# jcjones/ct-mapreduce

Hardware: AMD Instinct MI355X
Metric: certificates/sec whole-node + achieved HBM GB/s, 100M-entry synthetic CT batch (higher is better)
Workload: dtype u8

## Files before the change

ct_mapreduce_amd/csrc/der_walk.h:

```cpp
#pragma once
#include <stdint.h>

#include <type_traits>
#include <utility>

#if defined(__HIPCC__)
#define CTMR_HD __host__ __device__ __forceinline__
#else
#define CTMR_HD inline
#endif

namespace ctmr {

struct Walk {
  uint32_t serial_off, serial_len;
  int64_t not_before, not_after;
  uint32_t cn_off, cn_len;
  uint32_t spki_off, spki_len;
  bool bc_valid, is_ca;
  uint32_t nonfatal;
  uint32_t serial_w[5];
  bool cn_match;
  uint32_t meta_issuer, meta_crl;
  uint32_t issuer_name, subject_name;
// ... 1371 lines not shown
    uint32_t d0 = 0, d1 = 0;
    o.subject_name = q;
    q = walk_name<false, STRINGS>(r, L, q, tbs_end, ok, d0, d1, o.nonfatal, strings);
#endif
  }
  if constexpr (NAMES_ONLY) return ok;
  CTMR_STAGE(4);
  touch_all(r, q, SPKI_HEAD_NEED);
  rd_hdr(r, L, q, tbs_end, ok, tag, cs, ce);
  ok = ok & (tag == 0x30u);
  o.spki_off = q;
  o.spki_len = ce - q;
  AlgView key_alg{0u, 0u, 0u, 0u, 0u, 0u};
  KeyPending key_pending;
  key_pending.alg = PK_OTHER;
  {
    uint32_t k, tk, ck, ek;
    alg_id(r, L, cs, ce, ok, k, key_alg);
    rd_hdr(r, L, k, ce, ok, tk, ck, ek);
    ok = ok & (tk == 0x03u);
    bit_string_check(r, L, ck, ek - ck, ok);
    if (spki) spki_key_begin(r, L, key_alg, ck, ek, ok, o.nonfatal, key_pending);
  }
  q = ce;
  r.touch_tail(q, tbs_end);
  if (spki) {
    key_tail_of(r, q, key_pending);
    EcPending ecp;
    spki_key_finish<EC_DEFER>(r, L, key_alg, key_pending, ok, o.nonfatal, ecp);
    o.ec_curve = ecp.curve; o.ec_pos = ecp.pos; o.ec_shift = ecp.shift;
  }
  CTMR_STAGE(5);
  uint32_t nt = 0u;
  uint32_t san_cv = 0u, san_ev = 0u;
  (void)san_cv; (void)san_ev;
  if (ok & (q < tbs_end)) {
    rd_hdr<false>(r, L, q, tbs_end, ok, tag, cs, ce);
    nt = ok ? tag : 0u;
  }
  if (nt == 0x81u) {
    ok = ok & (ce <= tbs_end);
    bit_string_check(r, L, cs, ce - cs, ok);
    q = ce;
    nt = 0u;
    if (ok & (q < tbs_end)) {
      rd_hdr<false>(r, L, q, tbs_end, ok, tag, cs, ce);
      nt = ok ? tag : 0u;
    }
  }
  if (nt == 0x82u) {
    ok = ok & (ce <= tbs_end);
    bit_string_check(r, L, cs, ce - cs, ok);
    q = ce;
    nt = 0u;
    if (ok & (q < tbs_end)) {
      rd_hdr<false>(r, L, q, tbs_end, ok, tag, cs, ce);
      nt = ok ? tag : 0u;
    }
  }
  if ((nt == 0xa3u) | (nt == 0x83u)) ok = ok & (ce != cs);
  if (ok & (nt == 0xa3u)) {
    uint32_t e, e_end;
    r.touch(q, 48);
    rd_hdr<false>(r, L, cs, tbs_end, ok, tag, e, e_end);
    ok = ok & ((tag != 0x30u) | (e_end <= tbs_end));
    e_end = tag == 0x30u ? e_end : e;
    while (ok & (e < e_end)) {
      uint32_t t1, x, x_end, to, co, eo, tv, cv, ev, oidw;
      r.touch(e, 16);
      const uint32_t w0 = ldc(r, e, L), w1 = ldc(r, e + 4u, L), w2 = ldc(r, e + 8u, L);
      const bool p0 = ((w0 & 0xffff80ffu) == 0x03060030u) & ((w1 & 0x808080u) == 0u);
      const uint32_t b7 = w1 >> 24, b9 = (w2 >> 8) & 0xffu;
      const bool nc = p0 & (b7 == 0x04u) & ((w2 & 0x80u) == 0u);
      const bool cr = p0 & (b7 == 0x01u) & ((w2 & 0x80ff00ffu) == 0x00040001u) & ((b9 == 0x00u) | (b9 == 0xffu));
      if (nc | cr) {
        x_end = e + 2u + ((w0 >> 8) & 0xffu);
        co = e + 4u;
        eo = e + 7u;
        oidw = w1;
        cv = e + (cr ? 12u : 9u);
        ev = cv + (cr ? (w2 >> 24) : (w2 & 0xffu));
        ok = ok & (x_end <= e_end) & (ev <= x_end);
      } else {
        r.touch(e, 24);
        rd_hdr(r, L, e, e_end, ok, t1, x, x_end);
        rd_hdr(r, L, x, x_end, ok, to, co, eo);
        oidw = ldc(r, co, L);
        rd_hdr(r, L, eo, x_end, ok, tv, cv, ev);
        ok = ok & (t1 == 0x30u) & (to == 0x06u);
        ok = ok && oid_arcs_ok(r, L, co, eo);
        if (tv == 0x01u) {
          const uint32_t bv = ldc(r, cv, L) & 0xffu;
          ok = ok & (ev - cv == 1u) & ((bv == 0x00u) | (bv == 0xffu));
          rd_hdr(r, L, ev, x_end, ok, tv, cv, ev);
        }
        ok = ok & (tv == 0x04u);
      }
      {
        const bool is_crl = (eo - co == 3u) & ((oidw & 0xffffffu) == 0x1f1d55u);
        const uint32_t pk = o.meta_crl == META_NONE ? meta_pack(cv, ev - cv) : META_HOST;
        o.meta_crl = is_crl ? pk : o.meta_crl;
      }
      if constexpr (STRINGS) {
        if (ext & ok) {
          const uint32_t kind = ext_kind(eo - co, oidw, ldc(r, co + 4u, L));
          if ((kind >= 1u) & (kind <= 6u)) {
            ext_body_check(r, L, kind, cv, ev, ok);
          } else if (kind == 7u) {
            if constexpr (has_coop_refill<R>::value) {
              if ((san_ev == 0u) & (ev > cv)) { san_cv = cv; san_ev = ev; }
              else ext_san_check(r, L, cv, ev, ok, o.nonfatal);
            } else {
              ext_san_check(r, L, cv, ev, ok, o.nonfatal);
            }
          } else if (kind == 9u) {
            uint32_t uo[1] = {0u}, ul[1] = {0u}, nu = 0u;
            r.touch(cv, ev - cv < 200u ? ev - cv : 200u);
            crl_dps<false, true, STRINGS, 1u>(r, L, cv, ev, ok, uo, ul, nu, o.nonfatal, strings);
          } else if (kind == 8u) {
            if constexpr (has_defer_exact<R>::value) r.defer_exact();
            else ext_nc_check(r, L, cv, ev, ok);
          } else if ((kind >= 12u) & ext_nf) {
            if constexpr (has_defer_exact<R>::value) r.defer_exact();
            else o.nonfatal = (kind == 12u ? ext_ipaddr_ok(r, L, cv, ev) : ext_asnum_ok(r, L, cv, ev)) ? o.nonfatal : (o.nonfatal | WALK_NF_EXT);
          } else if ((kind == 10u) & ext_nf && ((ldc(r, co + 8u, L) & 0xffffu) == 0x0204u)) {
            if constexpr (has_defer_exact<R>::value) r.defer_exact();
            else o.nonfatal = ext_sct_ok(r, L, cv, ev) ? o.nonfatal : (o.nonfatal | WALK_NF_EXT);
          }
        }
      }
      if (ok & (eo - co == 3u) & ((oidw & 0xffffffu) == 0x131d55u)) {
        uint32_t tb, c, c_end, tf = 0u, cf = 0u, ef = 0u;
        rd_hdr(r, L, cv, ev, ok, tb, c, c_end);
        ok = ok & (tb == 0x30u) & (c_end == ev);
        bool ca = false;
        if (ok & (c < c_end)) {
          rd_hdr<false>(r, L, c, c_end, ok, tf, cf, ef);
          if (tf == 0x01u) {
            const uint32_t bv = ldc(r, cf, L) & 0xffu;
            ok = ok & (ef <= c_end) & (ef - cf == 1u) & ((bv == 0x00u) | (bv == 0xffu));
            ca = bv == 0xffu;
            c = ef;
            tf = 0u;
            if (ok & (c < c_end)) rd_hdr<false>(r, L, c, c_end, ok, tf, cf, ef);
          }
          if (ok & (c < c_end) & (tf == 0x02u)) {
            ok = ok & (ef <= c_end);
            int32_check(r, L, cf, ef - cf, ok, o.nonfatal);
          }
        }
        o.bc_valid = true;
        o.is_ca = ca;
      }
      e = x_end;
    }
  }
  if constexpr (STRINGS && has_coop_refill<R>::value) {
    if (ext) ext_san_coop(r, L, san_cv, ok ? san_ev : 0u, ok, o.nonfatal);
  }
  CTMR_STAGE(6);
  if constexpr (!TBS_ONLY) {
    const TailView<R> tv{r};
    uint32_t sq;
    alg_id(tv, L, tbs_end, L, ok, sq);
    rd_hdr(tv, L, sq, L, ok, tag, cs, ce);
    ok = ok & (tag == 0x03u);
    bit_string_check(tv, L, cs, ce - cs, ok);
// ... 19 lines not shown
```

ct_mapreduce_amd/csrc/engine/map.inc:

```

int ctmr_set_filter(ctmr_engine* e, const char* filter, size_t len, int log_expired, int64_t now) {
  if (!e || (len && !filter)) return CTMR_E_INVAL;
  std::lock_guard<std::mutex> g(e->mu);
  HIPCHK(e, hipSetDevice(e->device));
  FilterDev f;
  memset(&f, 0, sizeof f);
  f.active = len != 0;
  f.log_expired = log_expired != 0;
  f.now = now;
  f.strict_spki = e->strict_spki ? 1u : 0u;
  f.strict_strings = e->strict_strings ? 1u : 0u;
  f.strict_ext = e->strict_ext ? 1u : 0u;
  size_t s = 0;
  uint32_t nw = 0;
  for (;;) {
    size_t t = s;
    while (t < len && filter[t] != ',') t++;
    const size_t pl = t - s;
    if (f.n_pieces >= 64 || nw + (pl + 3) / 4 > 1024)
      return fail(e, CTMR_E_INVAL, "issuerCNFilter too large (max 64 pieces / 4096 bytes)");
    f.piece_len[f.n_pieces] = (uint32_t)pl;
    f.piece_word[f.n_pieces] = nw;
    memcpy((uint8_t*)(f.words + nw), filter + s, pl);
    nw += (uint32_t)((pl + 3) / 4);
// ... 36 lines not shown
  if (variant == 15 && !fuse) variant = 13;
  const dim3 grid((unsigned)((n + 63) / 64));
#ifdef CTMR_SWEEP
  static const size_t extra_lds = getenv("CTMR_EXTRA_LDS") ? (size_t)atoi(getenv("CTMR_EXTRA_LDS")) : 0;
#else
  constexpr size_t extra_lds = 0;
#endif
  const bool strict = e->strict_strings || e->strict_ext;
  if (variant == 15) {
    MetaCheck mc{};
    XchgArgs xa{};
    if (xchg) xa = *xchg;
    bool meta = false;
    if (e->cfg.collect_meta && e->d_meta_slots) {
      mc.slots = e->d_meta_slots; mc.mask = e->n_meta_slots - 1; mc.arena = e->d_meta_arena;
      mc.hour_pages = e->d_meta_hour_pages; mc.n_hour_pages = e->d_meta_hour_pages ? (uint32_t)e->meta_hour_pages.size() : 0u;
      mc.refs = e->d_meta_refs; mc.n_refs = e->max_issuers;
      mc.enabled = 1;
      meta = true;
      e->meta_precheck_n = first + n;
      e->meta_precheck_ent = fuse->ent - first;
    }
#define CTMR_LAUNCH_FUSED(META, MODE)                                                                                        \
  do {                                                                                                                       \
    if (strict)                                                                                                              \
      hipLaunchKernelGGL((k_map_fused<WIN_CH_STRICT, META, MODE, true>), grid, dim3(64),                                     \
                         WinGeo<WIN_CH_STRICT>::LDS_BYTES + extra_lds, e->stream, ma, *fuse, mc, xa);                        \
    else                                                                                                                     \
      hipLaunchKernelGGL((k_map_fused<WIN_CH_FAST, META, MODE, false>), grid, dim3(64),                                      \
                         WinGeo<WIN_CH_FAST>::LDS_BYTES + extra_lds, e->stream, ma, *fuse, mc, xa);                          \
  } while (0)
    if (mode == XM_OWNER) { if (meta) CTMR_LAUNCH_FUSED(true, XM_OWNER); else CTMR_LAUNCH_FUSED(false, XM_OWNER); }
    else if (mode == XM_BLOOM) { if (meta) CTMR_LAUNCH_FUSED(true, XM_BLOOM); else CTMR_LAUNCH_FUSED(false, XM_BLOOM); }
    else { if (meta) CTMR_LAUNCH_FUSED(true, XM_LOCAL); else CTMR_LAUNCH_FUSED(false, XM_LOCAL); }
#undef CTMR_LAUNCH_FUSED
  } else if (variant == 13) {
    if (strict) hipLaunchKernelGGL((k_map_winc<WIN_CH_STRICT, true>), grid, dim3(64), WinGeo<WIN_CH_STRICT>::LDS_BYTES + extra_lds, e->stream, ma);
    else hipLaunchKernelGGL((k_map_winc<WIN_CH_FAST, false>), grid, dim3(64), WinGeo<WIN_CH_FAST>::LDS_BYTES + extra_lds, e->stream, ma);
#ifdef CTMR_SWEEP
  } else if (variant == 2) {
    hipLaunchKernelGGL(k_map_direct, dim3((unsigned)((n + 255) / 256)), dim3(256), 0, e->stream, ma);
  } else if (variant == 1 && !d_ends) {
    uint32_t C = e->cfg.certs_per_tile ? e->cfg.certs_per_tile : 32;
    if (C > 64) C = 64;
    uint32_t lds = e->cfg.lds_tile_bytes ? e->cfg.lds_tile_bytes : 65536;
    if (lds > 160 * 1024) lds = 160 * 1024;
    ma.certs_per_tile = C; ma.lds_bytes = lds;
    if (!e->tile_attr_set) {
      HIPCHK(e, hipFuncSetAttribute((const void*)k_map_tile, hipFuncAttributeMaxDynamicSharedMemorySize, 160 * 1024));
      e->tile_attr_set = true;
    }
    hipLaunchKernelGGL(k_map_tile, dim3((unsigned)((n + C - 1) / C)), dim3(64), lds, e->stream, ma);
#endif
  } else {
    return fail(e, CTMR_E_INVAL, "map_variant %u is not built into this library", variant);
  }
  return CTMR_OK;
}

static bool round_fused(const ctmr_engine* e) { return e->cfg.map_variant == 0 || e->cfg.map_variant == 15; }

static void round_insert_args(ctmr_engine* e, const RoundCtx& rc, InsertArgs& ia) {
  ia.records = rc.d_records; ia.payload = rc.d_payload; ia.offsets = rc.d_offsets; ia.ends = rc.d_ends; ia.canon = e->d_canon;
  ia.t = e->tbl(); ia.ref0 = rc.ref0; ia.slot_id = (uint32_t*)e->d_scratch[SC_SLOTID];
  ia.ent = (uint32_t*)e->d_scratch[SC_ENT]; ia.n = rc.n; ia.stats = e->d_stats; ia.ord_base = rc.ord_base;
  ia.keypos = (const unsigned long long*)e->d_scratch[SC_KEYPOS]; ia.stage = nullptr; ia.bloom = nullptr; ia.bloom_wmask = 0;
}

static int round_prepare(ctmr_engine* e, RoundCtx& rc) {
  HIPCHK(e, hipSetDevice(e->device));
  e->rd.valid = false;
  const uint64_t n = rc.n;
  if (n >= 0xfffffff0ull) return fail(e, CTMR_E_INVAL, "batch too large (n < 2^32-16)");
  if (((uintptr_t)rc.d_payload & 15) != 0) return fail(e, CTMR_E_INVAL, "payload must be 16-byte aligned");
  int r;
  if (!rc.d_records) {
    if ((r = ensure(e, SC_RECORDS, n * sizeof(ctmr_record)))) return r;
    rc.d_records = (ctmr_record*)e->d_scratch[SC_RECORDS];
  }
  const uint64_t nb = (n + 1023) / 1024;
  if ((r = ensure(e, SC_SLOTID, n * 4))) return r;
  if ((r = ensure(e, SC_ENT, n * 4))) return r;
  if ((r = ensure(e, SC_BLKNEW, nb * 4))) return r;
  if ((r = ensure(e, SC_BLKBASE, nb * 8))) return r;
  if (e->strict_spki && n && (r = ensure(e, SC_KEYPOS, n * 8))) return r;
  if (e->cfg.collect_meta && (r = ensure(e, SC_META, n * 8))) return r;
  if ((r = ensure_capacity(e, n, true))) return r;
  rc.ref0 = e->arena_used;
  e->arena_used += n;
  e->epoch++;
  e->pairs_dirty = true;
  HIPCHK(e, hipMemsetAsync(e->d_stats, 0, 2 * sizeof(DevStats), e->stream));
  const bool fused = round_fused(e);
  if (!fused && rc.mode == XM_OWNER) return fail(e, CTMR_E_INVAL, "the owner-computes exchange needs the fused map kernel (map_variant 0 / 15)");
  if (rc.mode == XM_LOCAL && fused && e->d_bloom) {
    rc.mode = XM_BLOOM;
  }
  if (rc.mode == XM_BLOOM && !e->d_bloom) return fail(e, CTMR_E_INVAL, "ctmr_bloom_config has not been called");
  return CTMR_OK;
}

static int round_launch_range(ctmr_engine* e, RoundCtx& rc, const XchgArgs* xchg, uint64_t lo, uint64_t hi) {
  const uint64_t n = hi - lo;
  if (!n) return CTMR_OK;
  const bool prof = e->cfg.profile != 0;
  int r;
  InsertArgs ia;
  round_insert_args(e, rc, ia);
  ia.records += lo; ia.offsets += lo; ia.slot_id += lo; ia.ent += lo; ia.n = n; ia.ref0 += lo; ia.ord_base += (uint32_t)lo;
  if (ia.ends) ia.ends += lo;
  if (ia.keypos) ia.keypos += lo;
  const bool fused = round_fused(e);
  XchgArgs xa{};
  if (xchg) xa = *xchg;
  if (xa.stage) xa.stage += lo;
  if (xa.wave_cnt) xa.wave_cnt += (lo / 64) * MAX_WORLD;
  if (rc.mode == XM_BLOOM) {
    xa.bloom = e->d_bloom;
    xa.bloom_wmask = e->bloom_words - 1;
  }
  if (prof && lo == 0) HIPCHK(e, hipEventRecord(e->ev[0], e->stream));
  const int kmode = !fused ? XM_LOCAL : (rc.mode == XM_OWNER && rc.world == 1) ? XM_LOCAL : rc.mode;
  if ((r = launch_map(e, rc.d_payload, rc.d_offsets + lo, rc.d_issuer_idx + lo, rc.d_entry_type ? rc.d_entry_type + lo : nullptr, n,
                      rc.d_records + lo, true, fused ? &ia : nullptr, rc.d_ends ? rc.d_ends + lo : nullptr,
                      rc.blob_bytes + CTMR_PAYLOAD_PAD, kmode, &xa, lo)))
    return r;
  if (prof && hi == rc.n) HIPCHK(e, hipEventRecord(e->ev[1], e->stream));
  if (!fused) hipLaunchKernelGGL(k_insert, dim3((unsigned)((n + 255) / 256)), dim3(256), 0, e->stream, ia);
  if (e->strict_spki) {
    ia.stage = (kmode == XM_OWNER) ? xa.stage : nullptr;
    ia.bloom = (rc.mode == XM_BLOOM && fused) ? xa.bloom : nullptr;
    ia.bloom_wmask = xa.bloom_wmask;
    hipLaunchKernelGGL(k_ec_resolve<true>, dim3((unsigned)((n + EC_PER_BLOCK - 1) / EC_PER_BLOCK)), dim3(256), 0, e->stream, ia, rc.d_records + lo);
    hipLaunchKernelGGL(k_ec_resolve<false>, dim3((unsigned)((n + EC_PER_BLOCK - 1) / EC_PER_BLOCK)), dim3(256), 0, e->stream, ia, rc.d_records + lo);
  }
  hipLaunchKernelGGL(k_insert2, dim3((unsigned)((n + INSERT2_PER_BLOCK - 1) / INSERT2_PER_BLOCK)), dim3(256), 0, e->stream, ia, rc.d_records + lo);
  if (!fused && rc.mode == XM_BLOOM)
    hipLaunchKernelGGL(k_bloom_add, dim3((unsigned)((n + 255) / 256)), dim3(256), 0, e->stream, ia, e->d_bloom, e->bloom_words - 1);
  if (prof && hi == rc.n) HIPCHK(e, hipEventRecord(e->ev[2], e->stream));
  return CTMR_OK;
}

static int round_begin(ctmr_engine* e, RoundCtx& rc, const XchgArgs* xchg) {
  int r;
  if ((r = round_prepare(e, rc))) return r;
  return round_launch_range(e, rc, xchg, 0, rc.n);
}

static void round_compact(ctmr_engine* e, const RoundCtx& rc) {
  const uint64_t nb = (rc.n + 1023) / 1024;
  uint32_t* d_blk_new = (uint32_t*)e->d_scratch[SC_BLKNEW];
  uint64_t* d_blk_base = (uint64_t*)e->d_scratch[SC_BLKBASE];
  hipLaunchKernelGGL(k_scan_blocks, dim3(1), dim3(1024), 0, e->stream, d_blk_new, nb, d_blk_base);
  hipLaunchKernelGGL(k_compact, dim3((unsigned)nb), dim3(256), 0, e->stream, (const ctmr_record*)rc.d_records,
                     (const uint32_t*)e->d_scratch[SC_ENT], rc.n, (const uint64_t*)d_blk_base, rc.d_new_idx);
}

static int round_resolve(ctmr_engine* e, RoundCtx& rc, bool compact_now) {
  const bool prof = e->cfg.profile != 0;
  const uint64_t nb = (rc.n + 1023) / 1024;
  ResolveArgs ra;
  ra.ent = (uint32_t*)e->d_scratch[SC_ENT]; ra.issuer_counts = e->issuer_counts; ra.stats = e->d_stats;
  ra.blk_new = (uint32_t*)e->d_scratch[SC_BLKNEW]; ra.n = rc.n;
  hipLaunchKernelGGL(k_resolve, dim3((unsigned)(nb < 512 ? nb : 512)), dim3(1024), 0, e->stream, ra, nb);
  if (prof) HIPCHK(e, hipEventRecord(e->ev[3], e->stream));
  rc.compacted = false;
  if (compact_now && rc.d_new_idx) {
    round_compact(e, rc);
    rc.compacted = true;
  }
  if (prof) HIPCHK(e, hipEventRecord(e->ev[4], e->stream));
  return CTMR_OK;
}

static int round_collect(ctmr_engine* e, RoundCtx& rc) {
  const uint64_t n = rc.n;
  uint32_t* d_ent = (uint32_t*)e->d_scratch[SC_ENT];
  uint32_t* d_blk_new = (uint32_t*)e->d_scratch[SC_BLKNEW];
  DevStats both[2];
  uint64_t ends[2] = {0, rc.blob_bytes};
  HIPCHK(e, hipMemcpyAsync(both, e->d_stats, sizeof both, hipMemcpyDeviceToHost, e->stream));
  if (!rc.d_ends && rc.payload_bytes_known == ~0ull) {
    HIPCHK(e, hipMemcpyAsync(&ends[0], rc.d_offsets, 8, hipMemcpyDeviceToHost, e->stream));
    HIPCHK(e, hipMemcpyAsync(&ends[1], rc.d_offsets + n, 8, hipMemcpyDeviceToHost, e->stream));
  } else if (!rc.d_ends) {
    ends[1] = rc.payload_bytes_known;
  }
  HIPCHK(e, hipStreamSynchronize(e->stream));
  HIPCHK(e, hipGetLastError());
  rc.hs = both[0];
  rc.remote_new = both[1].n_new;
  rc.payload_bytes = ends[1] - ends[0];
  e->occupied += (rc.own_counted ? 0ull : rc.hs.n_new - rc.hs.n_remote) + rc.remote_new;
  if (rc.hs.n_full || both[1].n_full)
    return fail(e, CTMR_E_FULL, "known-certificate table full (%llu slots): %llu entries dropped",
                (unsigned long long)e->nslots, rc.hs.n_full + both[1].n_full);

  rc.host_new = 0;
  rc.host_list.clear();
  if (rc.hs.n_host) {
    std::vector<uint32_t> ent(n);
    HIPCHK(e, hipMemcpy(ent.data(), d_ent, n * 4, hipMemcpyDeviceToHost));
    for (uint64_t i = 0; i < n; i++) {
      if (((ent[i] >> 3) & 7u) != ES_HOST) continue;
      uint64_t off[2];
      ctmr_record rec;
      HIPCHK(e, hipMemcpy(off, rc.d_offsets + i, rc.d_ends ? 8 : 16, hipMemcpyDeviceToHost));
      if (rc.d_ends) HIPCHK(e, hipMemcpy(off + 1, rc.d_ends + i, 8, hipMemcpyDeviceToHost));
      HIPCHK(e, hipMemcpy(&rec, rc.d_records + i, sizeof rec, hipMemcpyDeviceToHost));
      std::vector<uint8_t> der(off[1] - off[0] + 32);
      HIPCHK(e, hipMemcpy(der.data(), rc.d_payload + off[0], off[1] - off[0], hipMemcpyDeviceToHost));
      HostReader hr{der.data()};
      Walk w;
      if (!walk_cert(hr, (uint32_t)(off[1] - off[0]), w, nullptr, e->strict_spki)) continue;
      const uint32_t canon = e->issuers[rec.issuer_idx].canon;
      std::string key = make_key(e, rec.exp_hour, canon);
      std::string member((const char*)der.data() + w.serial_off, w.serial_len);
      if (e->hstore[key].insert(member).second) {
        rc.host_new++;
        e->host_issuer_counts[canon]++;
        rc.host_list.push_back({i, rec.exp_hour, canon, member});
        uint8_t fl = rec.flags | CTMR_FL_WAS_UNKNOWN;
        HIPCHK(e, hipMemcpy((uint8_t*)(rc.d_records + i) + 1, &fl, 1, hipMemcpyHostToDevice));
        const uint32_t en = (ent[i] & ~(7u << 3)) | (ES_CLAIMED << 3);
        HIPCHK(e, hipMemcpy(d_ent + i, &en, 4, hipMemcpyHostToDevice));
        uint32_t bn;
        HIPCHK(e, hipMemcpy(&bn, d_blk_new + i / 1024, 4, hipMemcpyDeviceToHost));
        bn++;
        HIPCHK(e, hipMemcpy(d_blk_new + i / 1024, &bn, 4, hipMemcpyHostToDevice));
      }
    }
    if (rc.host_new && rc.compacted) {
      round_compact(e, rc);
      HIPCHK(e, hipStreamSynchronize(e->stream));
      HIPCHK(e, hipGetLastError());
    }
  }
  return CTMR_OK;
}

static int round_host_drop(ctmr_engine* e, RoundCtx& rc, const std::vector<size_t>& which) {
  if (which.empty()) return CTMR_OK;
  uint32_t* d_ent = (uint32_t*)e->d_scratch[SC_ENT];
  uint32_t* d_blk_new = (uint32_t*)e->d_scratch[SC_BLKNEW];
  for (size_t idx : which) {
    const RoundCtx::HostNew& h = rc.host_list[idx];
    const std::string key = make_key(e, h.exp_hour, h.canon);
    auto it = e->hstore.find(key);
    if (it != e->hstore.end()) {
      it->second.erase(h.member);
      if (it->second.empty()) e->hstore.erase(it);
    }
    auto ic = e->host_issuer_counts.find(h.canon);
// ... 112 lines not shown
```

ct_mapreduce_amd/csrc/kernels/readers.h:

```cpp
#pragma once
#include "../ctmr_dev.h"
#include "../entry_decode.h"
#include "../synth.h"

namespace ctmr {

struct __attribute__((packed, aligned(1))) U16t { uint32_t a, b, c, d; };

typedef uint32_t ctmr_u32x4 __attribute__((ext_vector_type(4)));
__device__ __forceinline__ uint4 ld_payload16(const uint4* p) {
  const ctmr_u32x4 t = __builtin_nontemporal_load((const ctmr_u32x4*)p);
  return make_uint4(t.x, t.y, t.z, t.w);
}
__device__ __forceinline__ void st_stream16(uint4* p, const uint4& v) {
  ctmr_u32x4 t;
  t.x = v.x; t.y = v.y; t.z = v.z; t.w = v.w;
  __builtin_nontemporal_store(t, (ctmr_u32x4*)p);
}
extern __shared__ __attribute__((aligned(16))) uint8_t smem[];
#ifndef CTMR_WIN_CH_FAST
#define CTMR_WIN_CH_FAST 13
#endif
#ifndef CTMR_WIN_CH_STRICT
#define CTMR_WIN_CH_STRICT 14
#endif
constexpr int WIN_CH_FAST = CTMR_WIN_CH_FAST, WIN_CH_STRICT = CTMR_WIN_CH_STRICT;
#ifndef CTMR_SAN_ALIGN
#define CTMR_SAN_ALIGN 32u
#endif
#ifndef CTMR_WIN_XDW14
#define CTMR_WIN_XDW14 0u
#endif
template <int WCH>
struct WinGeo {
  static constexpr uint32_t XDW = WCH == 13 ? 2u : WCH == 14 ? CTMR_WIN_XDW14 : 0u;
  static constexpr uint32_t WBYTES = (uint32_t)WCH * 16u + XDW * 4u;
  static constexpr uint32_t STRIDE = WCH == 16 ? 272u : WCH == 15 ? 248u : WCH == 13 ? 220u : (uint32_t)WCH * 16u + 12u;
#ifdef CTMR_WIN_NO_SKIP
  static constexpr uint32_t SKIP = 0u;
#else
  static constexpr uint32_t SKIP = WCH == 13 ? 8u : 0u;
#endif
  static constexpr uint32_t LDS_BYTES = 64u * STRIDE;
  static constexpr uint32_t ALIGN = STRIDE % 16u == 0u ? 16u : STRIDE % 8u == 0u ? 8u : 4u;
};
constexpr uint32_t WIN_LDS_MAX = WinGeo<WIN_CH_STRICT>::LDS_BYTES > WinGeo<WIN_CH_FAST>::LDS_BYTES ? WinGeo<WIN_CH_STRICT>::LDS_BYTES
                                                                                               : WinGeo<WIN_CH_FAST>::LDS_BYTES;
template <int WCH>
__device__ __forceinline__ uint32_t win_off(uint32_t c) { return c * WinGeo<WCH>::STRIDE; }
typedef uint32_t ctmr_u32x4_a16 __attribute__((ext_vector_type(4), aligned(16)));
typedef uint32_t ctmr_u32x4_a8 __attribute__((ext_vector_type(4), aligned(8)));
typedef uint32_t ctmr_u32x4_a4 __attribute__((ext_vector_type(4), aligned(4)));
typedef uint32_t ctmr_u32x2_a4 __attribute__((ext_vector_type(2), aligned(4)));
template <int WCH>
__device__ __forceinline__ void st_chunk(uint8_t* at, const uint4& v) {
  using vec_t = typename std::conditional<WinGeo<WCH>::ALIGN == 16u, ctmr_u32x4_a16,
                                          typename std::conditional<WinGeo<WCH>::ALIGN == 8u, ctmr_u32x4_a8, ctmr_u32x4_a4>::type>::type;
  vec_t t;
  t.x = v.x; t.y = v.y; t.z = v.z; t.w = v.w;
  *(vec_t*)at = t;
}
template <int WCH>
__device__ __forceinline__ void st_part(uint8_t* at, const uint4& v) {
  if constexpr (WinGeo<WCH>::XDW == 2u) {
    ctmr_u32x2_a4 t;
    t.x = v.x; t.y = v.y;
    *(ctmr_u32x2_a4*)at = t;
  } else if constexpr (WinGeo<WCH>::XDW == 1u) {
    *(uint32_t*)at = v.x;
  } else if constexpr (WinGeo<WCH>::XDW == 3u) {
    ctmr_u32x2_a4 t;
    t.x = v.x; t.y = v.y;
    *(ctmr_u32x2_a4*)at = t;
    *(uint32_t*)(at + 8) = v.z;
  }
}
__device__ __forceinline__ void st_half(uint8_t* at, uint32_t x, uint32_t y) {
  ctmr_u32x2_a4 t;
  t.x = x; t.y = y;
  *(ctmr_u32x2_a4*)at = t;
}
template <int WCH>
constexpr uint32_t win_loaders() { return (uint32_t)WCH + (WinGeo<WCH>::XDW ? 1u : 0u); }

constexpr uint32_t REL_NONE = 0x80000000u;
constexpr uint64_t REL_SPAN = 0x7e000000ull;
struct WaveBuf {
  __amdgpu_buffer_rsrc_t rs;
  uint64_t b128;
};
__device__ __forceinline__ WaveBuf wave_buf(const uint8_t* payload, uint64_t limit, uint64_t lo0) {
  const uint32_t l = __builtin_amdgcn_readfirstlane((uint32_t)lo0), h = __builtin_amdgcn_readfirstlane((uint32_t)(lo0 >> 32));
  const uint64_t b128 = (((uint64_t)h << 32) | l) & ~127ull;
  uint64_t span = limit > b128 ? limit - b128 : 0ull;
  span = span > 0x7fffffffull ? 0x7fffffffull : span;
  return WaveBuf{__builtin_amdgcn_make_buffer_rsrc((void*)(payload + b128), 0, (int)span, 0x00020000), b128};
}
__device__ __forceinline__ uint32_t wave_rel(const WaveBuf& wb, uint64_t lo, bool has) {
  const uint64_t d = lo - wb.b128;
  return (has & (lo >= wb.b128) & (d < REL_SPAN)) ? (uint32_t)d : REL_NONE;
}
template <bool NT = true>
__device__ __forceinline__ uint4 ld_chunk(const WaveBuf& wb, uint32_t off) {
  const ctmr_u32x4 t = __builtin_amdgcn_raw_buffer_load_b128(wb.rs, (int)off, 0, NT ? 2  : 0);
  return make_uint4(t.x, t.y, t.z, t.w);
}

// ... 311 lines not shown
```

ct_mapreduce_amd/csrc/kernels/reduce.h:

```cpp
#pragma once
#include "keyrec.h"
#include "map.h"

namespace ctmr {

#define AGENT __HIP_MEMORY_SCOPE_AGENT

__device__ __forceinline__ unsigned long long ld_agent(const unsigned long long* p) {
  return __hip_atomic_load(p, __ATOMIC_RELAXED, AGENT);
}
__device__ __forceinline__ void st_agent(unsigned long long* p, unsigned long long v) {
  __hip_atomic_store(p, v, __ATOMIC_RELAXED, AGENT);
}

__device__ __forceinline__ bool cell_equals(const KeyCell* c, unsigned long long meta, const unsigned long long s[5]) {
  bool eq = (ld_agent(&c->meta) & ~CELL_SHADOW) == meta;
#pragma unroll
  for (int k = 0; k < 5; k++) eq = eq && ld_agent(&c->s[k]) == s[k];
  return eq;
}
__device__ __forceinline__ void cell_write(KeyCell* c, unsigned long long meta, const unsigned long long s[5], uint32_t ord) {
  uint4* q = (uint4*)c;
  q[0] = make_uint4((uint32_t)meta, (uint32_t)(meta >> 32), (uint32_t)s[0], (uint32_t)(s[0] >> 32));
  q[1] = make_uint4((uint32_t)s[1], (uint32_t)(s[1] >> 32), (uint32_t)s[2], (uint32_t)(s[2] >> 32));
// ... 487 lines not shown
      const uint4 r0 = rp[0], r1 = rp[1];
      bool good;
      if constexpr (P256) {
        good = ec_point_bits<CurveP256>((const uint32_t*)a.payload, xbit);
      } else {
        switch (curve) {
          case 2u: good = ec_point_bits<CurveP384>((const uint32_t*)a.payload, xbit); break;
          case 3u: good = ec_point_bits<CurveP521>((const uint32_t*)a.payload, xbit); break;
          case 4u: good = ec_point_bits<CurveP224>((const uint32_t*)a.payload, xbit); break;
          default: good = ec_point_bits<CurveP192>((const uint32_t*)a.payload, xbit); break;
        }
      }
      if (!good) {
        const uint32_t stn = (r0.x & 0xffu) == CTMR_ST_ENTRY_DECODE_ERROR ? (uint32_t)CTMR_ST_ENTRY_DECODE_ERROR : (uint32_t)CTMR_ST_PARSE_ERROR;
        rp[0] = make_uint4(stn | (((r0.x >> 8) & CTMR_FL_PRECERT) << 8), 0u, r0.z, 0u);
        rp[1] = make_uint4(0u, 0u, 0u, 0u);
        if ((kp >> 38) & 1ull) {
          a.stage[(i & ~63ull) + ((kp >> 39) & 63ull)].meta = 0ull;
        } else if (ent_state(e) == ES_REMOTE) {
          atomicAdd(&a.stats->n_xl, ~0ull);
        }
        a.ent[i] = ent_pack(stn, ES_NONE, e >> 8);
      } else if (ent_state(e) != ES_PENDING) {
        a.ent[i] = e & ~ENT_KEY_PENDING;
      } else {
        unsigned long long s[5];
        record_key(a, i, r0, r1, s);
        const unsigned long long meta = key_meta((int32_t)r0.y, e >> 8, r0.x >> 16);
        const unsigned long long h = key_hash(meta, s);
        const uint32_t state = insert_probe_h(a, i, meta, s, h);
        if (state != ES_CLAIMED && state != ES_DEFER) {
          ((uint8_t*)(records + i))[1] = (uint8_t)((r0.x >> 8) & ~CTMR_FL_WAS_UNKNOWN);
        } else if (a.bloom) {
          uint64_t word;
          unsigned long long bits;
          bloom_pos(h, a.bloom_wmask, word, bits);
          atomicOr(&a.bloom[word], bits);
        }
        a.ent[i] = (e & ~(ENT_KEY_PENDING | (7u << 3))) | (state << 3);
      }
    }
  }
}

__device__ __forceinline__ void wave_agg_add(bool active, uint32_t key, unsigned long long* arr) {
  unsigned long long todo = __ballot(active);
  while (todo) {
    const int leader = __ffsll((long long)todo) - 1;
    const uint32_t k = __shfl(key, leader);
    const unsigned long long same = __ballot(active && key == k) & todo;
    if ((int)(threadIdx.x & 63) == leader) atomicAdd(&arr[k], (unsigned long long)__popcll(same));
    todo &= ~same;
  }
}

__device__ __forceinline__ bool pair_add(PairSlot* pairs, uint64_t pmask, unsigned long long key,
                                         long long delta) {
  uint64_t j = mixk(key) & pmask;
  for (uint64_t probes = 0; probes <= pmask; probes++) {
    unsigned long long k = ld_agent(&pairs[j].key);
    if (k == 0ull) {
      const unsigned long long old = atomicCAS(&pairs[j].key, 0ull, key);
      k = old == 0ull ? key : old;
    }
    if (k == key) {
      atomicAdd(&pairs[j].count, (unsigned long long)delta);
      return true;
    }
    j = (j + 1) & pmask;
  }
  return false;
}

struct ResolveArgs {
  const uint32_t* ent;
  unsigned long long* issuer_counts;
  DevStats* stats;
  uint32_t* blk_new;
  uint64_t n;
};

constexpr uint32_t RES_LDS_ISSUERS = 4096;

__global__ void __launch_bounds__(1024) k_resolve(ResolveArgs a, uint64_t nb) {
  __shared__ uint32_t hist[CTMR_ST__COUNT + 5];
  __shared__ uint32_t ih[RES_LDS_ISSUERS];
  __shared__ uint32_t blk_cnt[4];
  if (threadIdx.x < CTMR_ST__COUNT + 5) hist[threadIdx.x] = 0;
  for (uint32_t k = threadIdx.x; k < RES_LDS_ISSUERS; k += 1024) ih[k] = 0;
  __syncthreads();
  const uint64_t nsb = (nb + 3) / 4;
  for (uint64_t sb = blockIdx.x; sb < nsb; sb += gridDim.x) {
    if (threadIdx.x < 4) blk_cnt[threadIdx.x] = 0;
    __syncthreads();
    const uint64_t i0 = sb * 4096 + (uint64_t)threadIdx.x * 4u;
    uint32_t e[4] = {0xffffffffu, 0xffffffffu, 0xffffffffu, 0xffffffffu};
    bool live[4] = {false, false, false, false};
    if (i0 + 4 <= a.n) {
      const uint4 v = *(const uint4*)(a.ent + i0);
      e[0] = v.x; e[1] = v.y; e[2] = v.z; e[3] = v.w;
      live[0] = live[1] = live[2] = live[3] = true;
    } else {
      for (uint32_t k = 0; i0 + k < a.n; k++) {
        e[k] = a.ent[i0 + k];
        live[k] = true;
      }
    }
    uint32_t w_new = 0, w_dup = 0, w_host = 0, w_full = 0, w_rem = 0;
#pragma unroll
    for (uint32_t k = 0; k < 4; k++) {
      const uint32_t status = live[k] ? (e[k] & 7u) : (uint32_t)CTMR_ST__COUNT;
      const uint32_t st = ent_state(e[k]), canon = e[k] >> 8;
      bool is_new = live[k] & ((st == ES_CLAIMED) | (st == ES_DEFER));
      const bool is_remote = live[k] & (st == ES_REMOTE);
      if (is_new && canon < RES_LDS_ISSUERS) atomicAdd(&ih[canon], 1u);
      wave_agg_add(is_new && canon >= RES_LDS_ISSUERS, canon, a.issuer_counts);
      is_new = is_new | is_remote;
      w_new += (uint32_t)__popcll(__ballot(is_new));
      w_dup += (uint32_t)__popcll(__ballot(live[k] & (st == ES_DUP)));
      w_host += (uint32_t)__popcll(__ballot(live[k] & (st == ES_HOST)));
      w_full += (uint32_t)__popcll(__ballot(live[k] & (st == ES_FULL)));
      w_rem += (uint32_t)__popcll(__ballot(is_remote));
#pragma unroll
      for (uint32_t s = 0; s < CTMR_ST__COUNT; s++) {
        const unsigned long long m = __ballot(status == s);
        if ((threadIdx.x & 63) == 0 && m) atomicAdd(&hist[s], (uint32_t)__popcll(m));
      }
    }
    if ((threadIdx.x & 63) == 0) {
      if (w_rem) atomicAdd(&hist[CTMR_ST__COUNT + 4], w_rem);
      if (w_new) {
        atomicAdd(&blk_cnt[threadIdx.x >> 8], w_new);
        atomicAdd(&hist[CTMR_ST__COUNT], w_new);
      }
      if (w_dup) atomicAdd(&hist[CTMR_ST__COUNT + 1], w_dup);
      if (w_host) atomicAdd(&hist[CTMR_ST__COUNT + 2], w_host);
      if (w_full) atomicAdd(&hist[CTMR_ST__COUNT + 3], w_full);
    }
    __syncthreads();
    if (threadIdx.x < 4 && sb * 4 + threadIdx.x < nb) a.blk_new[sb * 4 + threadIdx.x] = blk_cnt[threadIdx.x];
  }
  __syncthreads();
  for (uint32_t k = threadIdx.x; k < RES_LDS_ISSUERS; k += 1024)
    if (ih[k]) atomicAdd(&a.issuer_counts[k], (unsigned long long)ih[k]);
  if (threadIdx.x < CTMR_ST__COUNT) {
    if (hist[threadIdx.x]) atomicAdd(&a.stats->by_status[threadIdx.x], (unsigned long long)hist[threadIdx.x]);
  } else if (threadIdx.x == CTMR_ST__COUNT) {
    if (hist[CTMR_ST__COUNT]) atomicAdd(&a.stats->n_new, (unsigned long long)hist[CTMR_ST__COUNT]);
  } else if (threadIdx.x == CTMR_ST__COUNT + 1) {
    if (hist[CTMR_ST__COUNT + 1]) atomicAdd(&a.stats->n_dup, (unsigned long long)hist[CTMR_ST__COUNT + 1]);
  } else if (threadIdx.x == CTMR_ST__COUNT + 2) {
    if (hist[CTMR_ST__COUNT + 2]) atomicAdd(&a.stats->n_host, (unsigned long long)hist[CTMR_ST__COUNT + 2]);
  } else if (threadIdx.x == CTMR_ST__COUNT + 3) {
    if (hist[CTMR_ST__COUNT + 3]) atomicAdd(&a.stats->n_full, (unsigned long long)hist[CTMR_ST__COUNT + 3]);
  } else if (threadIdx.x == CTMR_ST__COUNT + 4) {
    if (hist[CTMR_ST__COUNT + 4]) atomicAdd(&a.stats->n_remote, (unsigned long long)hist[CTMR_ST__COUNT + 4]);
  }
}

__global__ void __launch_bounds__(256) k_compact(const ctmr_record* records, const uint32_t* ent, uint64_t n,
                                                 const uint64_t* blk_base, uint64_t* new_idx) {
  __shared__ uint32_t wave_cnt[4];
  const uint64_t i0 = (uint64_t)blockIdx.x * 1024 + threadIdx.x * 4u;
  const uint32_t lane = threadIdx.x & 63, wv = threadIdx.x >> 6;
  bool f[4] = {false, false, false, false};
  if (ent) {
    if (i0 + 4 <= n) {
      const uint4 v = *(const uint4*)(ent + i0);
      f[0] = ent_is_new(v.x); f[1] = ent_is_new(v.y); f[2] = ent_is_new(v.z); f[3] = ent_is_new(v.w);
    } else {
      for (uint32_t k = 0; k < 4 && i0 + k < n; k++) f[k] = ent_is_new(ent[i0 + k]);
    }
  } else {
#pragma unroll
    for (uint32_t k = 0; k < 4; k++)
      if (i0 + k < n) f[k] = (((const uint8_t*)(records + i0 + k))[1] & CTMR_FL_WAS_UNKNOWN) != 0;
  }
  const uint32_t c = (uint32_t)f[0] + f[1] + f[2] + f[3];
  const unsigned long long m0 = __ballot(c & 1u), m1 = __ballot(c & 2u), m2 = __ballot(c & 4u);
  const unsigned long long lt = (1ull << lane) - 1ull;
  uint32_t pre = (uint32_t)__popcll(m0 & lt) + 2u * (uint32_t)__popcll(m1 & lt) + 4u * (uint32_t)__popcll(m2 & lt);
  if (lane == 0) wave_cnt[wv] = (uint32_t)__popcll(m0) + 2u * (uint32_t)__popcll(m1) + 4u * (uint32_t)__popcll(m2);
  __syncthreads();
  if (c) {
    for (uint32_t k = 0; k < wv; k++) pre += wave_cnt[k];
    uint64_t at = blk_base[blockIdx.x] + pre;
#pragma unroll
    for (uint32_t k = 0; k < 4; k++)
      if (f[k]) new_idx[at++] = i0 + k;
  }
}

__global__ void __launch_bounds__(1024) k_scan_blocks(const uint32_t* blk_new, uint64_t nb,
                                                      uint64_t* blk_base) {
  __shared__ unsigned long long wsum[16];
  const uint32_t lane = threadIdx.x & 63u, wv = threadIdx.x >> 6;
  unsigned long long carry = 0;
  for (uint64_t base = 0; base < nb; base += 4096u) {
    const uint64_t i0 = base + (uint64_t)threadIdx.x * 4u;
    uint32_t v[4];
#pragma unroll
    for (uint32_t k = 0; k < 4; k++) v[k] = i0 + k < nb ? blk_new[i0 + k] : 0u;
    const unsigned long long tsum = (unsigned long long)v[0] + v[1] + v[2] + v[3];
    unsigned long long x = tsum;
#pragma unroll
    for (int d = 1; d < 64; d <<= 1) {
      const unsigned long long y = __shfl_up(x, d);
      if ((int)lane >= d) x += y;
    }
    if (lane == 63u) wsum[wv] = x;
    __syncthreads();
    unsigned long long before = 0, all = 0;
#pragma unroll
    for (uint32_t k = 0; k < 16; k++) {
      if (k < wv) before += wsum[k];
      all += wsum[k];
    }
    unsigned long long run = carry + before + x - tsum;
#pragma unroll
    for (uint32_t k = 0; k < 4; k++) {
      if (i0 + k < nb) blk_base[i0 + k] = run;
      run += v[k];
    }
    carry += all;
    __syncthreads();
  }
}

constexpr uint32_t SCAN_TILE = 4096;

__device__ __forceinline__ unsigned long long block_exclusive_256(unsigned long long v, unsigned long long* total) {
  __shared__ unsigned long long wsum[4];
  const uint32_t lane = threadIdx.x & 63, wv = threadIdx.x >> 6;
  unsigned long long x = v;
#pragma unroll
  for (int d = 1; d < 64; d <<= 1) {
    const unsigned long long y = __shfl_up(x, d);
    if ((int)lane >= d) x += y;
  }
  __syncthreads();
  if (lane == 63) wsum[wv] = x;
  __syncthreads();
// ... 68 lines not shown
```

Measured before the change: 2.692 billion.

## Fuse resolve and compaction into single-pass decoupled-lookback scan kernel

Replaces the resolve, block-scan and compact sequence with a single kernel, k_resolve_compact. It takes superblocks through an atomic ticket and computes the global offsets of new entries with a decoupled lookback over agent-scope flags, then writes new_idx directly. This removes two kernel launches, the single-block serial scan, and the second read of the ent array. It adds a memset, extra lookback slots, and spin-waiting that depends on forward progress. The diff also trims the DER walk touch window from 24 to 20 bytes and the strict window channel count from 14 to 13.

Result: faster. 2.745 billion (median of 6 runs) (+2.0%).

```diff
diff --git a/ct_mapreduce_amd/csrc/der_walk.h b/ct_mapreduce_amd/csrc/der_walk.h
--- a/ct_mapreduce_amd/csrc/der_walk.h
+++ b/ct_mapreduce_amd/csrc/der_walk.h
@@ -1477,7 +1477,7 @@
         ev = cv + (cr ? (w2 >> 24) : (w2 & 0xffu));
         ok = ok & (x_end <= e_end) & (ev <= x_end);
       } else {
-        r.touch(e, 24);
+        r.touch(e, 20);
         rd_hdr(r, L, e, e_end, ok, t1, x, x_end);
         rd_hdr(r, L, x, x_end, ok, to, co, eo);
         oidw = ldc(r, co, L);
diff --git a/ct_mapreduce_amd/csrc/engine/map.inc b/ct_mapreduce_amd/csrc/engine/map.inc
--- a/ct_mapreduce_amd/csrc/engine/map.inc
+++ b/ct_mapreduce_amd/csrc/engine/map.inc
@@ -142,7 +142,7 @@
   if ((r = ensure(e, SC_SLOTID, n * 4))) return r;
   if ((r = ensure(e, SC_ENT, n * 4))) return r;
   if ((r = ensure(e, SC_BLKNEW, nb * 4))) return r;
-  if ((r = ensure(e, SC_BLKBASE, nb * 8))) return r;
+  if ((r = ensure(e, SC_BLKBASE, (nb + 2) * 8))) return r;
   if (e->strict_spki && n && (r = ensure(e, SC_KEYPOS, n * 8))) return r;
   if (e->cfg.collect_meta && (r = ensure(e, SC_META, n * 8))) return r;
   if ((r = ensure_capacity(e, n, true))) return r;
@@ -222,13 +222,17 @@
   ResolveArgs ra;
   ra.ent = (uint32_t*)e->d_scratch[SC_ENT]; ra.issuer_counts = e->issuer_counts; ra.stats = e->d_stats;
   ra.blk_new = (uint32_t*)e->d_scratch[SC_BLKNEW]; ra.n = rc.n;
-  hipLaunchKernelGGL(k_resolve, dim3((unsigned)(nb < 512 ? nb : 512)), dim3(1024), 0, e->stream, ra, nb);
-  if (prof) HIPCHK(e, hipEventRecord(e->ev[3], e->stream));
   rc.compacted = false;
   if (compact_now && rc.d_new_idx) {
-    round_compact(e, rc);
+    const uint64_t nsb = (nb + 3) / 4;
+    unsigned long long* d_look = (unsigned long long*)e->d_scratch[SC_BLKBASE];
+    HIPCHK(e, hipMemsetAsync(d_look, 0, (nsb + 1) * 8, e->stream));
+    hipLaunchKernelGGL(k_resolve_compact, dim3((unsigned)(nsb < 512 ? nsb : 512)), dim3(1024), 0, e->stream, ra, nb, d_look, rc.d_new_idx);
     rc.compacted = true;
-  }
+  } else {
+    hipLaunchKernelGGL(k_resolve, dim3((unsigned)(nb < 512 ? nb : 512)), dim3(1024), 0, e->stream, ra, nb);
+  }
+  if (prof) HIPCHK(e, hipEventRecord(e->ev[3], e->stream));
   if (prof) HIPCHK(e, hipEventRecord(e->ev[4], e->stream));
   return CTMR_OK;
 }
diff --git a/ct_mapreduce_amd/csrc/kernels/readers.h b/ct_mapreduce_amd/csrc/kernels/readers.h
--- a/ct_mapreduce_amd/csrc/kernels/readers.h
+++ b/ct_mapreduce_amd/csrc/kernels/readers.h
@@ -22,7 +22,7 @@
 #define CTMR_WIN_CH_FAST 13
 #endif
 #ifndef CTMR_WIN_CH_STRICT
-#define CTMR_WIN_CH_STRICT 14
+#define CTMR_WIN_CH_STRICT 13
 #endif
 constexpr int WIN_CH_FAST = CTMR_WIN_CH_FAST, WIN_CH_STRICT = CTMR_WIN_CH_STRICT;
 #ifndef CTMR_SAN_ALIGN
diff --git a/ct_mapreduce_amd/csrc/kernels/reduce.h b/ct_mapreduce_amd/csrc/kernels/reduce.h
--- a/ct_mapreduce_amd/csrc/kernels/reduce.h
+++ b/ct_mapreduce_amd/csrc/kernels/reduce.h
@@ -593,65 +593,56 @@
 
 constexpr uint32_t RES_LDS_ISSUERS = 4096;
 
-__global__ void __launch_bounds__(1024) k_resolve(ResolveArgs a, uint64_t nb) {
-  __shared__ uint32_t hist[CTMR_ST__COUNT + 5];
-  __shared__ uint32_t ih[RES_LDS_ISSUERS];
-  __shared__ uint32_t blk_cnt[4];
-  if (threadIdx.x < CTMR_ST__COUNT + 5) hist[threadIdx.x] = 0;
-  for (uint32_t k = threadIdx.x; k < RES_LDS_ISSUERS; k += 1024) ih[k] = 0;
-  __syncthreads();
-  const uint64_t nsb = (nb + 3) / 4;
-  for (uint64_t sb = blockIdx.x; sb < nsb; sb += gridDim.x) {
-    if (threadIdx.x < 4) blk_cnt[threadIdx.x] = 0;
-    __syncthreads();
-    const uint64_t i0 = sb * 4096 + (uint64_t)threadIdx.x * 4u;
-    uint32_t e[4] = {0xffffffffu, 0xffffffffu, 0xffffffffu, 0xffffffffu};
-    bool live[4] = {false, false, false, false};
-    if (i0 + 4 <= a.n) {
-      const uint4 v = *(const uint4*)(a.ent + i0);
-      e[0] = v.x; e[1] = v.y; e[2] = v.z; e[3] = v.w;
-      live[0] = live[1] = live[2] = live[3] = true;
-    } else {
-      for (uint32_t k = 0; i0 + k < a.n; k++) {
-        e[k] = a.ent[i0 + k];
-        live[k] = true;
-      }
-    }
-    uint32_t w_new = 0, w_dup = 0, w_host = 0, w_full = 0, w_rem = 0;
-#pragma unroll
-    for (uint32_t k = 0; k < 4; k++) {
-      const uint32_t status = live[k] ? (e[k] & 7u) : (uint32_t)CTMR_ST__COUNT;
-      const uint32_t st = ent_state(e[k]), canon = e[k] >> 8;
-      bool is_new = live[k] & ((st == ES_CLAIMED) | (st == ES_DEFER));
-      const bool is_remote = live[k] & (st == ES_REMOTE);
-      if (is_new && canon < RES_LDS_ISSUERS) atomicAdd(&ih[canon], 1u);
-      wave_agg_add(is_new && canon >= RES_LDS_ISSUERS, canon, a.issuer_counts);
-      is_new = is_new | is_remote;
-      w_new += (uint32_t)__popcll(__ballot(is_new));
-      w_dup += (uint32_t)__popcll(__ballot(live[k] & (st == ES_DUP)));
-      w_host += (uint32_t)__popcll(__ballot(live[k] & (st == ES_HOST)));
-      w_full += (uint32_t)__popcll(__ballot(live[k] & (st == ES_FULL)));
-      w_rem += (uint32_t)__popcll(__ballot(is_remote));
-#pragma unroll
-      for (uint32_t s = 0; s < CTMR_ST__COUNT; s++) {
-        const unsigned long long m = __ballot(status == s);
-        if ((threadIdx.x & 63) == 0 && m) atomicAdd(&hist[s], (uint32_t)__popcll(m));
-      }
-    }
-    if ((threadIdx.x & 63) == 0) {
-      if (w_rem) atomicAdd(&hist[CTMR_ST__COUNT + 4], w_rem);
-      if (w_new) {
-        atomicAdd(&blk_cnt[threadIdx.x >> 8], w_new);
-        atomicAdd(&hist[CTMR_ST__COUNT], w_new);
-      }
-      if (w_dup) atomicAdd(&hist[CTMR_ST__COUNT + 1], w_dup);
-      if (w_host) atomicAdd(&hist[CTMR_ST__COUNT + 2], w_host);
-      if (w_full) atomicAdd(&hist[CTMR_ST__COUNT + 3], w_full);
-    }
-    __syncthreads();
-    if (threadIdx.x < 4 && sb * 4 + threadIdx.x < nb) a.blk_new[sb * 4 + threadIdx.x] = blk_cnt[threadIdx.x];
-  }
-  __syncthreads();
+__device__ __forceinline__ uint32_t resolve_tally(const ResolveArgs& a, const uint32_t (&e)[4], const bool (&live)[4], uint32_t* hist,
+                                                  uint32_t* ih) {
+  uint32_t w_new = 0, w_dup = 0, w_host = 0, w_full = 0, w_rem = 0;
+#pragma unroll
+  for (uint32_t k = 0; k < 4; k++) {
+    const uint32_t status = live[k] ? (e[k] & 7u) : (uint32_t)CTMR_ST__COUNT;
+    const uint32_t st = ent_state(e[k]), canon = e[k] >> 8;
+    bool is_new = live[k] & ((st == ES_CLAIMED) | (st == ES_DEFER));
+    const bool is_remote = live[k] & (st == ES_REMOTE);
+    if (is_new && canon < RES_LDS_ISSUERS) atomicAdd(&ih[canon], 1u);
+    wave_agg_add(is_new && canon >= RES_LDS_ISSUERS, canon, a.issuer_counts);
+    is_new = is_new | is_remote;
+    w_new += (uint32_t)__popcll(__ballot(is_new));
+    w_dup += (uint32_t)__popcll(__ballot(live[k] & (st == ES_DUP)));
+    w_host += (uint32_t)__popcll(__ballot(live[k] & (st == ES_HOST)));
+    w_full += (uint32_t)__popcll(__ballot(live[k] & (st == ES_FULL)));
+    w_rem += (uint32_t)__popcll(__ballot(is_remote));
+#pragma unroll
+    for (uint32_t s = 0; s < CTMR_ST__COUNT; s++) {
+      const unsigned long long m = __ballot(status == s);
+      if ((threadIdx.x & 63) == 0 && m) atomicAdd(&hist[s], (uint32_t)__popcll(m));
+    }
+  }
+  if ((threadIdx.x & 63) == 0) {
+    if (w_rem) atomicAdd(&hist[CTMR_ST__COUNT + 4], w_rem);
+    if (w_new) atomicAdd(&hist[CTMR_ST__COUNT], w_new);
+    if (w_dup) atomicAdd(&hist[CTMR_ST__COUNT + 1], w_dup);
+    if (w_host) atomicAdd(&hist[CTMR_ST__COUNT + 2], w_host);
+    if (w_full) atomicAdd(&hist[CTMR_ST__COUNT + 3], w_full);
+  }
+  return w_new;
+}
+__device__ __forceinline__ void resolve_load(const ResolveArgs& a, uint64_t i0, uint32_t (&e)[4], bool (&live)[4]) {
+#pragma unroll
+  for (uint32_t k = 0; k < 4; k++) {
+    e[k] = 0xffffffffu;
+    live[k] = false;
+  }
+  if (i0 + 4 <= a.n) {
+    const uint4 v = *(const uint4*)(a.ent + i0);
+    e[0] = v.x; e[1] = v.y; e[2] = v.z; e[3] = v.w;
+    live[0] = live[1] = live[2] = live[3] = true;
+  } else {
+    for (uint32_t k = 0; i0 + k < a.n; k++) {
+      e[k] = a.ent[i0 + k];
+      live[k] = true;
+    }
+  }
+}
+__device__ __forceinline__ void resolve_flush(const ResolveArgs& a, const uint32_t* hist, const uint32_t* ih) {
   for (uint32_t k = threadIdx.x; k < RES_LDS_ISSUERS; k += 1024)
     if (ih[k]) atomicAdd(&a.issuer_counts[k], (unsigned long long)ih[k]);
   if (threadIdx.x < CTMR_ST__COUNT) {
@@ -669,6 +660,103 @@
   }
 }
 
+__global__ void __launch_bounds__(1024) k_resolve(ResolveArgs a, uint64_t nb) {
+  __shared__ uint32_t hist[CTMR_ST__COUNT + 5];
+  __shared__ uint32_t ih[RES_LDS_ISSUERS];
+  __shared__ uint32_t blk_cnt[4];
+  if (threadIdx.x < CTMR_ST__COUNT + 5) hist[threadIdx.x] = 0;
+  for (uint32_t k = threadIdx.x; k < RES_LDS_ISSUERS; k += 1024) ih[k] = 0;
+  __syncthreads();
+  const uint64_t nsb = (nb + 3) / 4;
+  for (uint64_t sb = blockIdx.x; sb < nsb; sb += gridDim.x) {
+    if (threadIdx.x < 4) blk_cnt[threadIdx.x] = 0;
+    __syncthreads();
+    uint32_t e[4];
+    bool live[4];
+    resolve_load(a, sb * 4096 + (uint64_t)threadIdx.x * 4u, e, live);
+    const uint32_t w_new = resolve_tally(a, e, live, hist, ih);
+    if ((threadIdx.x & 63) == 0 && w_new) atomicAdd(&blk_cnt[threadIdx.x >> 8], w_new);
+    __syncthreads();
+    if (threadIdx.x < 4 && sb * 4 + threadIdx.x < nb) a.blk_new[sb * 4 + threadIdx.x] = blk_cnt[threadIdx.x];
+  }
+  __syncthreads();
+  resolve_flush(a, hist, ih);
+}
+
+constexpr unsigned long long LB_AGG = 1ull << 62, LB_PREFIX = 2ull << 62, LB_VAL = (1ull << 62) - 1ull;
+__global__ void __launch_bounds__(1024) k_resolve_compact(ResolveArgs a, uint64_t nb, unsigned long long* look, uint64_t* new_idx) {
+  __shared__ uint32_t hist[CTMR_ST__COUNT + 5];
+  __shared__ uint32_t ih[RES_LDS_ISSUERS];
+  __shared__ uint32_t wave_cnt[16];
+  __shared__ unsigned long long s_step, s_base;
+  if (threadIdx.x < CTMR_ST__COUNT + 5) hist[threadIdx.x] = 0;
+  for (uint32_t k = threadIdx.x; k < RES_LDS_ISSUERS; k += 1024) ih[k] = 0;
+  const uint64_t nsb = (nb + 3) / 4;
+  const uint32_t lane = threadIdx.x & 63u, wv = threadIdx.x >> 6;
+  for (;;) {
+    if (threadIdx.x == 0) s_step = atomicAdd(&look[nsb], 1ull);
+    __syncthreads();
+    const uint64_t sb = s_step;
+    if (sb >= nsb) break;
+    const uint64_t i0 = sb * 4096 + (uint64_t)threadIdx.x * 4u;
+    uint32_t e[4];
+    bool live[4];
+    resolve_load(a, i0, e, live);
+    bool f[4];
+#pragma unroll
+    for (uint32_t k = 0; k < 4; k++) f[k] = live[k] & ent_is_new(e[k]);
+    const uint32_t c = (uint32_t)f[0] + f[1] + f[2] + f[3];
+    const unsigned long long m0 = __ballot(c & 1u), m1 = __ballot(c & 2u), m2 = __ballot(c & 4u);
+    const unsigned long long lt = (1ull << lane) - 1ull;
+    const uint32_t pre = (uint32_t)__popcll(m0 & lt) + 2u * (uint32_t)__popcll(m1 & lt) + 4u * (uint32_t)__popcll(m2 & lt);
+    if (lane == 0) wave_cnt[wv] = (uint32_t)__popcll(m0) + 2u * (uint32_t)__popcll(m1) + 4u * (uint32_t)__popcll(m2);
+    __syncthreads();
+    uint32_t before = 0, total = 0;
+#pragma unroll
+    for (uint32_t k = 0; k < 16; k++) {
+      const uint32_t t = wave_cnt[k];
+      before += k < wv ? t : 0u;
+      total += t;
+    }
+    if (wv == 0) {
+      unsigned long long excl = 0ull;
+      if (sb == 0) {
+        if (lane == 0) st_agent(&look[0], LB_PREFIX | total);
+      } else {
+        if (lane == 0) st_agent(&look[sb], LB_AGG | total);
+        for (uint64_t j = sb;; j -= 64u) {
+          unsigned long long w = LB_PREFIX;
+          if (j > lane) {
+            while (((w = ld_agent(&look[j - 1u - lane])) >> 62) == 0ull) __builtin_amdgcn_s_sleep(1);
+          }
+          const unsigned long long pm = __ballot((w >> 62) == 2ull);
+          const uint32_t upto = pm ? (uint32_t)(__ffsll((long long)pm) - 1) : 63u;
+          unsigned long long v = lane <= upto ? (w & LB_VAL) : 0ull;
+#pragma unroll
+          for (int d = 32; d > 0; d >>= 1) v += __shfl_xor(v, d);
+          excl += v;
+          if (pm) break;
+        }
+        if (lane == 0) st_agent(&look[sb], LB_PREFIX | (excl + total));
+      }
+      if (lane == 0) s_base = excl;
+    }
+    if (threadIdx.x < 4 && sb * 4 + threadIdx.x < nb)
+      a.blk_new[sb * 4 + threadIdx.x] = wave_cnt[4 * threadIdx.x] + wave_cnt[4 * threadIdx.x + 1] + wave_cnt[4 * threadIdx.x + 2] +
+                                        wave_cnt[4 * threadIdx.x + 3];
+    (void)resolve_tally(a, e, live, hist, ih);
+    __syncthreads();
+    if (c) {
+      uint64_t at = s_base + before + pre;
+#pragma unroll
+      for (uint32_t k = 0; k < 4; k++)
+        if (f[k]) new_idx[at++] = i0 + k;
+    }
+  }
+  __syncthreads();
+  resolve_flush(a, hist, ih);
+}
+
 __global__ void __launch_bounds__(256) k_compact(const ctmr_record* records, const uint32_t* ent, uint64_t n,
                                                  const uint64_t* blk_base, uint64_t* new_idx) {
   __shared__ uint32_t wave_cnt[4];
```
